# yenjane-dot/cognitive-aim-depth-estimation

Measured on NVIDIA B200. Metric: images/sec at 518x518 bf16, higher is better.
Workload: dtype bf16

## Files before the change

### cognitive_aim_depth_estimation_b200/csrc/common.cuh

```cuda
#pragma once

#include <cuda.h>
#include <cuda_bf16.h>
#include <cuda_runtime.h>
#include <stdint.h>
#include <stdio.h>

namespace ca {

enum : int {
  CA_OK = 0,
  CA_ERR_INVALID = 1,
  CA_ERR_CUDA = 2,
  CA_ERR_UNSUPPORTED = 3
};

__device__ __forceinline__ uint32_t smem_u32(const void* p) {
  return static_cast<uint32_t>(__cvta_generic_to_shared(p));
}
__device__ __forceinline__ uint32_t lane_id() { return threadIdx.x & 31u; }
__device__ __forceinline__ uint32_t warp_id() { return threadIdx.x >> 5; }

__device__ __forceinline__ bool elect_one_sync() {
  uint32_t pred;
// ... 163 lines not shown
    if ((++spins & 0x3fu) == 0 && (clock64() - t0) > 4000000000LL) {
      printf("[cogaim] mbarrier wait timed out: block (%d,%d,%d) thread %d bar@%u parity %u\n", blockIdx.x,
             blockIdx.y, blockIdx.z, threadIdx.x, smem_u32(bar), parity);
      __trap();
    }
  }
}

__device__ __forceinline__ void tma_prefetch_desc(const CUtensorMap* tm) {
  asm volatile("prefetch.tensormap [%0];" ::"l"(reinterpret_cast<uint64_t>(tm)) : "memory");
}
__device__ __forceinline__ void tma_load_2d(void* smem_dst, const CUtensorMap* tm, uint64_t* bar, int c0, int c1) {
  asm volatile(
      "cp.async.bulk.tensor.2d.shared::cluster.global.mbarrier::complete_tx::bytes [%0], [%1, {%3, %4}], [%2];"
      ::"r"(smem_u32(smem_dst)),
      "l"(reinterpret_cast<uint64_t>(tm)), "r"(smem_u32(bar)), "r"(c0), "r"(c1)
      : "memory");
}
__device__ __forceinline__ void tma_load_3d(void* smem_dst, const CUtensorMap* tm, uint64_t* bar, int c0, int c1,
                                            int c2) {
  asm volatile(
      "cp.async.bulk.tensor.3d.shared::cluster.global.mbarrier::complete_tx::bytes [%0], [%1, {%3, %4, %5}], [%2];"
      ::"r"(smem_u32(smem_dst)),
      "l"(reinterpret_cast<uint64_t>(tm)), "r"(smem_u32(bar)), "r"(c0), "r"(c1), "r"(c2)
      : "memory");
}

__device__ __forceinline__ void tma_reduce_add_2d(const CUtensorMap* tm, const void* smem_src, int c0, int c1) {
  asm volatile("cp.reduce.async.bulk.tensor.2d.global.shared::cta.add.tile.bulk_group [%0, {%2, %3}], [%1];" ::"l"(
                   reinterpret_cast<uint64_t>(tm)),
               "r"(smem_u32(smem_src)), "r"(c0), "r"(c1)
               : "memory");
}
__device__ __forceinline__ void bulk_commit_group() { asm volatile("cp.async.bulk.commit_group;" ::: "memory"); }
template <int kPending>
__device__ __forceinline__ void bulk_wait_group_read() {
  asm volatile("cp.async.bulk.wait_group.read %0;" ::"n"(kPending) : "memory");
}
template <int kPending>
__device__ __forceinline__ void bulk_wait_group() {
  asm volatile("cp.async.bulk.wait_group %0;" ::"n"(kPending) : "memory");
}

__device__ __forceinline__ void tmem_alloc(uint32_t* smem_result, uint32_t ncols) {
  asm volatile("tcgen05.alloc.cta_group::1.sync.aligned.shared::cta.b32 [%0], %1;" ::"r"(smem_u32(smem_result)),
               "r"(ncols)
               : "memory");
  asm volatile("tcgen05.relinquish_alloc_permit.cta_group::1.sync.aligned;" ::: "memory");
}
__device__ __forceinline__ void tmem_dealloc(uint32_t taddr, uint32_t ncols) {
  asm volatile("tcgen05.dealloc.cta_group::1.sync.aligned.b32 %0, %1;" ::"r"(taddr), "r"(ncols) : "memory");
}
__device__ __forceinline__ void tc_fence_before() { asm volatile("tcgen05.fence::before_thread_sync;" ::: "memory"); }
__device__ __forceinline__ void tc_fence_after() { asm volatile("tcgen05.fence::after_thread_sync;" ::: "memory"); }

__device__ __forceinline__ void umma_bf16(uint32_t tmem_d, uint64_t adesc, uint64_t bdesc, uint32_t idesc,
                                          uint32_t accumulate) {
  asm volatile(
      "{\n\t.reg .pred p;\n\t"
      "setp.ne.b32 p, %4, 0;\n\t"
      "tcgen05.mma.cta_group::1.kind::f16 [%0], %1, %2, %3, p;\n\t}"
      ::"r"(tmem_d),
      "l"(adesc), "l"(bdesc), "r"(idesc), "r"(accumulate)
      : "memory");
}
__device__ __forceinline__ void umma_bf16_ts(uint32_t tmem_d, uint32_t tmem_a, uint64_t bdesc, uint32_t idesc,
// ... 147 lines not shown
```

### cognitive_aim_depth_estimation_b200/csrc/gemm.cu

```cuda
#include "common.cuh"
#include "gemm.cuh"

#include <cuda_fp16.h>
#include "host.h"

#include <stdlib.h>

#ifndef CA_GEMM_RELEASE_ARRIVE
#define CA_GEMM_RELEASE_ARRIVE 0
#endif

namespace ca {

namespace {

constexpr int BM = 128;
constexpr int BK = 64;
constexpr int kNumEpiWarps = 8;
constexpr int kGemmThreads = (2 + kNumEpiWarps) * 32;
constexpr int kEpiStageBytes = 32 * 128;
__device__ __forceinline__ uint32_t epi_off(int r, int piece) { return r * 128 + ((piece ^ (r & 7)) << 4); }

template <int BN>
struct GemmCfg {
  static constexpr int kStages = (BN == 256) ? 4 : 6;
  static constexpr int kABytes = BM * BK * 2;
  static constexpr int kBBytes = BN * BK * 2;
  static constexpr int kStageBytes = kABytes + kBBytes;
  static constexpr int kTmemCols = 2 * BN;
  static constexpr int kStagingBytes = kNumEpiWarps * kEpiStageBytes;
  static constexpr int kSmemBytes = kStages * kStageBytes + kStagingBytes + 1024  + 256 ;
};

struct GemmKernelArgs {
  int M, N, K;
  int m_tiles, n_tiles, total_tiles;
  int w_batched;
  void* out;
  int ldo;
  long long out_batch_stride;
  const float* bias;
  const float* ls;
  const float* pos;
  int patches_per_img;
  float scale_log2;
  float* part_a;
  float* part_b;
  const float* col_max;
  const float* col_rinv;
  int partials;
  float2* ln_stats;
  int ln_slots;
  float ln_eps;
  __nv_bfloat16* shadow;
  int ld_shadow;
  int dbg;
};

__device__ __forceinline__ void gelu_erf2(float& x0, float& x1) {
  float s0, s1, p0, p1;
  fmul2(s0, s1, x0, x1, x0, x1);
  ffma2(p0, p1, s0, s1, 6.013480685629347e-11f, -5.644098521884189e-09f);
  ffma2v(p0, p1, p0, p1, s0, s1, 2.3467518417419342e-07f, 2.3467518417419342e-07f);
  ffma2v(p0, p1, p0, p1, s0, s1, -5.765378773503471e-06f, -5.765378773503471e-06f);
  ffma2v(p0, p1, p0, p1, s0, s1, 9.46131840464659e-05f, 9.46131840464659e-05f);
  ffma2v(p0, p1, p0, p1, s0, s1, -0.0011143309529870749f, -0.0011143309529870749f);
  ffma2v(p0, p1, p0, p1, s0, s1, 0.009830592200160027f, 0.009830592200160027f);
  ffma2v(p0, p1, p0, p1, s0, s1, -0.06636093556880951f, -0.06636093556880951f);
  ffma2v(p0, p1, p0, p1, s0, s1, 0.39890772104263306f, 0.39890772104263306f);
  const float phi0 = ffma_sat(p0, x0, 0.5f), phi1 = ffma_sat(p1, x1, 0.5f);
  fmul2(x0, x1, x0, x1, phi0, phi1);
}

__device__ __forceinline__ float ln_row_rstd(const GemmKernelArgs& p, int row) {
  if (row >= p.M) return 1.f;
  const float2* st = p.ln_stats + static_cast<size_t>(row) * p.ln_slots;
  const float inv_dim = 1.f / (128.f * p.ln_slots);
  float tot = 0.f, m2 = 0.f;
  for (int i = 0; i < p.ln_slots; ++i) {
    const float2 t = __ldg(st + i);
    tot += t.x;
    m2 += t.y;
  }
  const float mean = tot * inv_dim;
  for (int i = 0; i < p.ln_slots; ++i) {
    const float d = __ldg(st + i).x * (1.f / 128.f) - mean;
    m2 = fmaf(128.f * d, d, m2);
  }
  return rsqrtf(m2 * inv_dim + p.ln_eps);
}

template <int BN, int EPI>
__device__ __forceinline__ void epilogue_tile(const GemmKernelArgs& p, const CUtensorMap* tmap_x, uint32_t tmem_acc, int b,
                                              int mt, int nt, int quad, int half, uint8_t* stage, float rstd = 1.f) {
  constexpr int kSpan = BN / 2;
  const int lane = lane_id();
  const int row = mt * BM + quad * 32 + lane;
  const int col_base = nt * BN + half * kSpan;
  const bool row_ok = row < p.M;
  const uint32_t taddr = tmem_acc + (static_cast<uint32_t>(quad * 32) << 16) + static_cast<uint32_t>(half * kSpan);

  if constexpr (EPI == EPI_ROWSTATS) {
    constexpr int kSub = kSpan / 64;
    const uint32_t stage_s = smem_u32(stage);
#pragma unroll 1
    for (int sub = 0; sub < kSub; ++sub) {
      const int col_sub = col_base + sub * 64;
      const uint32_t taddr_sub = taddr + static_cast<uint32_t>(sub * 64);
      const bool full = col_sub + 64 <= p.N;
      float mx = -INFINITY;
#pragma unroll
      for (int c = 0; c < 64; c += 32) {
        uint32_t v[32];
        tmem_ld32(taddr_sub + c, v);
        tmem_ld_wait();
        if (full) {
          float m0 = __uint_as_float(v[0]), m1 = __uint_as_float(v[1]);
#pragma unroll
          for (int j = 2; j < 32; j += 2) {
            m0 = fmaxf(m0, __uint_as_float(v[j]));
            m1 = fmaxf(m1, __uint_as_float(v[j + 1]));
          }
          mx = fmaxf(mx, fmaxf(m0, m1));
        } else {
#pragma unroll
          for (int j = 0; j < 32; ++j)
            if (col_sub + c + j < p.N) mx = fmaxf(mx, __uint_as_float(v[j]));
// ... 59 lines not shown
      }
    }
    return;
  } else if constexpr (EPI == EPI_COLSUM) {
    const float* cmax = p.col_max + static_cast<size_t>(b) * p.N;
    const float* cinv = p.col_rinv + static_cast<size_t>(b) * p.N;
    float sum = 0.f;
#pragma unroll
    for (int c = 0; c < kSpan; c += 32) {
      uint32_t v[32];
      tmem_ld32(taddr + c, v);
      tmem_ld_wait();
#pragma unroll
      for (int j = 0; j < 32; ++j) {
        const int col = col_base + c + j;
        if (col < p.N) {
          const float s = __uint_as_float(v[j]) * p.scale_log2;
          sum += fast_exp2(s - __ldg(cmax + col)) * __ldg(cinv + col);
        }
      }
    }
    if (row_ok) {
      const size_t o = (static_cast<size_t>(b) * p.partials + nt * 2 + half) * p.M + row;
      p.part_a[o] = sum;
    }
    return;
  } else {
    const int lrow = lane >> 3;
    const int seg = lane & 7;
    const uint32_t stage_s = smem_u32(stage);
    if constexpr (EPI == EPI_BIAS_BF16 || EPI == EPI_GELU_BF16 || EPI == EPI_LN_BIAS_BF16 || EPI == EPI_LN_GELU_BF16) {
      constexpr bool kLn = (EPI == EPI_LN_BIAS_BF16 || EPI == EPI_LN_GELU_BF16);
      constexpr bool kGelu = (EPI == EPI_GELU_BF16 || EPI == EPI_LN_GELU_BF16);
#pragma unroll 1
      for (int c = 0; c < kSpan; c += 64) {
        const int col = col_base + c;
#pragma unroll
        for (int hh = 0; hh < 2; ++hh) {
          uint32_t v[32];
          tmem_ld32(taddr + c + 32 * hh, v);
          tmem_ld_wait();
          if (col < p.N) {
            const float4* b4 = reinterpret_cast<const float4*>(p.bias + col + 32 * hh);
#pragma unroll
            for (int j = 0; j < 4; ++j) {
              float a[8];
#pragma unroll
              for (int h = 0; h < 2; ++h) {
                const float4 t = __ldg(b4 + 2 * j + h);
                if constexpr (kLn) {
                  a[4 * h + 0] = fmaf(rstd, __uint_as_float(v[8 * j + 4 * h + 0]), t.x);
                  a[4 * h + 1] = fmaf(rstd, __uint_as_float(v[8 * j + 4 * h + 1]), t.y);
                  a[4 * h + 2] = fmaf(rstd, __uint_as_float(v[8 * j + 4 * h + 2]), t.z);
                  a[4 * h + 3] = fmaf(rstd, __uint_as_float(v[8 * j + 4 * h + 3]), t.w);
                } else {
                  a[4 * h + 0] = __uint_as_float(v[8 * j + 4 * h + 0]) + t.x;
                  a[4 * h + 1] = __uint_as_float(v[8 * j + 4 * h + 1]) + t.y;
                  a[4 * h + 2] = __uint_as_float(v[8 * j + 4 * h + 2]) + t.z;
                  a[4 * h + 3] = __uint_as_float(v[8 * j + 4 * h + 3]) + t.w;
                }
              }
              if constexpr (kGelu) {
#pragma unroll
                for (int i = 0; i < 8; i += 2) gelu_erf2(a[i], a[i + 1]);
              }
              uint4 w;
              w.x = pack_bf16x2(a[0], a[1]);
              w.y = pack_bf16x2(a[2], a[3]);
              w.z = pack_bf16x2(a[4], a[5]);
              w.w = pack_bf16x2(a[6], a[7]);
              sts128(stage_s + epi_off(lane, 4 * hh + j), w);
            }
          }
        }
        if (col < p.N) {
          __syncwarp();
          __nv_bfloat16* obase = reinterpret_cast<__nv_bfloat16*>(p.out) + static_cast<size_t>(b) * p.out_batch_stride +
                                 col + seg * 8;
#pragma unroll
          for (int i = 0; i < 8; ++i) {
            const int rr = lrow + 4 * i;
            const int grow = mt * BM + quad * 32 + rr;
            const uint4 w = lds128(stage_s + epi_off(rr, seg));
            if (grow < p.M) *reinterpret_cast<uint4*>(obase + static_cast<size_t>(grow) * p.ldo) = w;
          }
          __syncwarp();
        }
      }
    } else if constexpr (EPI == EPI_RESID_F32) {
      constexpr int kChunks = kSpan / 32;
#pragma unroll 1
      for (int g = 0; g < kChunks; ++g) {
        const int c = g * 32;
        uint32_t v[32];
        tmem_ld32(taddr + c, v);
        tmem_ld_wait();
        const int col = col_base + c;
        if (lane == 0) bulk_wait_group_read<0>();
        __syncwarp();
#pragma unroll
        for (int j = 0; j < 8; ++j) {
          const float4 t = __ldg(reinterpret_cast<const float4*>(p.bias + col) + j);
          const float4 l4 = __ldg(reinterpret_cast<const float4*>(p.ls + col) + j);
          sts128f(stage_s + epi_off(lane, j),
              make_float4(l4.x * (__uint_as_float(v[4 * j + 0]) + t.x), l4.y * (__uint_as_float(v[4 * j + 1]) + t.y),
                          l4.z * (__uint_as_float(v[4 * j + 2]) + t.z), l4.w * (__uint_as_float(v[4 * j + 3]) + t.w)));
        }
        fence_proxy_async_smem();
        __syncwarp();
        if (lane == 0) {
          tma_reduce_add_2d(tmap_x, stage, col, mt * BM + quad * 32);
          bulk_commit_group();
        }
      }
    } else {
#pragma unroll 1
      for (int c = 0; c < kSpan; c += 32) {
        uint32_t v[32];
        tmem_ld32(taddr + c, v);
        tmem_ld_wait();
        const int col = col_base + c;
        if (col < p.N) {
#pragma unroll
          for (int j = 0; j < 8; ++j) {
            float4 a = make_float4(__uint_as_float(v[4 * j + 0]), __uint_as_float(v[4 * j + 1]),
                                   __uint_as_float(v[4 * j + 2]), __uint_as_float(v[4 * j + 3]));
            if constexpr (EPI != EPI_F32) {
              const float4 t = __ldg(reinterpret_cast<const float4*>(p.bias + col) + j);
              a.x += t.x;
// ... 101 lines not shown
      uint32_t phase = 0;
      int acc = 0;
      uint32_t acc_phase = 0;
      for (int tile = blockIdx.x; tile < p.total_tiles; tile += gridDim.x) {
        mbar_wait(&acc_empty[acc], acc_phase ^ 1u);
        tc_fence_after();
        const uint32_t tmem_d = tmem_base + static_cast<uint32_t>(acc * BN);
        for (int kb = 0; kb < kblocks; ++kb) {
          mbar_wait(&full_bar[stage], phase);
          tc_fence_after();
          const uint64_t adesc = umma_smem_desc_sw128(smem_u32(smem_a + stage * Cfg::kABytes));
          const uint64_t bdesc = umma_smem_desc_sw128(smem_u32(smem_b + stage * Cfg::kBBytes));
#pragma unroll
          for (int k = 0; k < BK / 16; ++k) {
            umma_bf16(tmem_d, adesc + 2 * k, bdesc + 2 * k, idesc, (kb | k) != 0 ? 1u : 0u);
          }
          umma_commit(&empty_bar[stage]);
          if (++stage == Cfg::kStages) {
            stage = 0;
            phase ^= 1u;
          }
        }
        umma_commit(&acc_full[acc]);
        acc ^= 1;
        if (acc == 0) acc_phase ^= 1u;
      }
    }
  } else {
    const int e = warp - 2;
    const int quad = warp & 3;
    const int half = e >> 2;
    int acc = 0;
    uint32_t acc_phase = 0;
    for (int tile = blockIdx.x; tile < p.total_tiles; tile += gridDim.x) {
      const int nt = tile % p.n_tiles;
      const int rest = tile / p.n_tiles;
      const int mt = rest % p.m_tiles;
      const int b = rest / p.m_tiles;
      float rstd = 1.f;
      if constexpr (EPI == EPI_LN_BIAS_BF16 || EPI == EPI_LN_GELU_BF16) rstd = ln_row_rstd(p, mt * BM + quad * 32 + lane);
      mbar_wait(&acc_full[acc], acc_phase);
      tc_fence_after();
      epilogue_tile<BN, EPI>(p, &tmap_x, tmem_base + static_cast<uint32_t>(acc * BN), b, mt, nt, quad, half,
                             smem_stage + e * kEpiStageBytes, rstd);
      tc_fence_before();
      __syncwarp();
      if (lane == 0) mbar_arrive(&acc_empty[acc]);
      acc ^= 1;
      if (acc == 0) acc_phase ^= 1u;
    }
    if constexpr (EPI == EPI_RESID_F32) {
      if (lane == 0) bulk_wait_group<0>();
    }
  }

  tc_fence_before();
  __syncthreads();
  if (warp == 1) {
    tc_fence_after();
    tmem_dealloc(tmem_base, Cfg::kTmemCols);
  }
}

struct Gemm2Cfg {
  static constexpr int BN = 256;
  static constexpr int kStages = 6;
  static constexpr int kABytes = BM * BK * 2;
  static constexpr int kBBytes = (BN / 2) * BK * 2;
  static constexpr int kStageBytes = kABytes + kBBytes;
  static constexpr int kTmemCols = 2 * BN;
  static constexpr int kStagingBytes = kNumEpiWarps * kEpiStageBytes;
  static constexpr int kSmemBytes = kStages * kStageBytes + kStagingBytes + 1024 + 256;
};

template <int EPI>
__global__ void __cluster_dims__(2, 1, 1) __launch_bounds__(kGemmThreads, 1)
gemm2_tcgen05_kernel(const __grid_constant__ CUtensorMap tmap_a, const __grid_constant__ CUtensorMap tmap_w,
                     const __grid_constant__ CUtensorMap tmap_x, const GemmKernelArgs p) {
  using Cfg = Gemm2Cfg;
  constexpr int BN = Cfg::BN;
  constexpr bool kResidLn = (EPI == EPI_RESID_LN_F32);
  constexpr int n_stages = Cfg::kStages;
  constexpr int staging_bytes = Cfg::kStagingBytes;
  extern __shared__ uint8_t smem_raw[];
  uint8_t* smem = reinterpret_cast<uint8_t*>((reinterpret_cast<uintptr_t>(smem_raw) + 1023) & ~uintptr_t(1023));
  uint8_t* smem_a = smem;
  uint8_t* smem_b = smem + n_stages * Cfg::kABytes;
  uint8_t* smem_stage = smem + n_stages * Cfg::kStageBytes;
  uint64_t* bars = reinterpret_cast<uint64_t*>(smem_stage + staging_bytes);
  uint64_t* full_bar = bars;
  uint64_t* empty_bar = bars + Cfg::kStages;
  uint64_t* acc_full = bars + 2 * Cfg::kStages;
  uint64_t* acc_empty = acc_full + 2;
  uint32_t* tmem_slot = reinterpret_cast<uint32_t*>(acc_empty + 2);

  const int warp = warp_id();
  const int lane = lane_id();
  const uint32_t rank = cluster_ctarank();
  const int cluster_id = blockIdx.x >> 1;
  const int n_clusters = gridDim.x >> 1;
  const int kblocks = (p.K + BK - 1) / BK;

  if (warp == 0 && lane == 0) {
    tma_prefetch_desc(&tmap_a);
    tma_prefetch_desc(&tmap_w);
// ... 18 lines not shown
    if (lane == 0) {
      int stage = 0;
      uint32_t phase = 0;
      for (int tile = cluster_id; tile < p.total_tiles; tile += n_clusters) {
        const int nt = tile % p.n_tiles;
        const int rest = tile / p.n_tiles;
        const int mt2 = rest % p.m_tiles;
        const int b = rest / p.m_tiles;
        for (int kb = 0; kb < kblocks; ++kb) {
          mbar_wait(&empty_bar[stage], phase ^ 1u);
          const uint32_t leader_full = mapa_cluster(smem_u32(&full_bar[stage]), 0);
          const bool la = !(p.dbg & 2) || kb == 0, lb = !(p.dbg & 1) || kb == 0;
          const int mt_l = (p.dbg & 16) ? 0 : mt2, nt_l = (p.dbg & 16) ? 0 : nt;
          if (rank == 0)
            mbar_arrive_expect_tx(&full_bar[stage], 2 * ((la ? Cfg::kABytes : 0) + (lb ? Cfg::kBBytes : 0)));
          if (la) tma_load_3d_2sm(smem_a + stage * Cfg::kABytes, &tmap_a, leader_full, kb * BK, mt_l * 2 * BM + rank * BM, b);
          if (lb)
            tma_load_3d_2sm(smem_b + stage * Cfg::kBBytes, &tmap_w, leader_full, kb * BK, nt_l * BN + rank * (BN / 2),
                            p.w_batched ? b : 0);
          if (++stage == n_stages) {
            stage = 0;
            phase ^= 1u;
          }
        }
      }
    }
  } else if (warp == 1) {
    if (rank == 0 && lane == 0) {
      constexpr uint32_t idesc = umma_idesc_bf16(2 * BM, BN, 0, 0);
      int stage = 0;
      uint32_t phase = 0;
      int acc = 0;
      uint32_t acc_phase = 0;
      for (int tile = cluster_id; tile < p.total_tiles; tile += n_clusters) {
        mbar_wait(&acc_empty[acc], acc_phase ^ 1u);
        tc_fence_after();
        const uint32_t tmem_d = tmem_base + static_cast<uint32_t>(acc * BN);
        for (int kb = 0; kb < kblocks; ++kb) {
          mbar_wait(&full_bar[stage], phase);
          tc_fence_after();
          const uint64_t adesc = umma_smem_desc_sw128(smem_u32(smem_a + stage * Cfg::kABytes));
          const uint64_t bdesc = umma_smem_desc_sw128(smem_u32(smem_b + stage * Cfg::kBBytes));
#pragma unroll
          for (int k = 0; k < BK / 16; ++k) {
            umma_bf16_2sm(tmem_d, adesc + 2 * k, bdesc + 2 * k, idesc, (kb | k) != 0 ? 1u : 0u);
          }
          umma_commit_2sm(&empty_bar[stage], 3);
          if (++stage == n_stages) {
            stage = 0;
            phase ^= 1u;
          }
        }
        umma_commit_2sm(&acc_full[acc], 3);
        acc ^= 1;
        if (acc == 0) acc_phase ^= 1u;
      }
    }
  } else {
    const int e = warp - 2;
    const int quad = warp & 3;
    const int half = e >> 2;
    int acc = 0;
    uint32_t acc_phase = 0;
    if constexpr (kResidLn) {
      const int lrow = lane >> 3, seg = lane & 7;
      const uint32_t stage_s = smem_u32(smem_stage + e * kEpiStageBytes);
      const int my_tiles = cluster_id < p.total_tiles ? (p.total_tiles - cluster_id + n_clusters - 1) / n_clusters : 0;
      const int total_chunks = my_tiles * 4;
      auto tile_origin = [&](int i, int& col0, int& row0, int& nt) {
        const int tile = cluster_id + i * n_clusters;
        nt = tile % p.n_tiles;
        const int mt2 = (tile / p.n_tiles) % p.m_tiles;
        col0 = nt * BN + half * 128;
        row0 = (mt2 * 2 + static_cast<int>(rank)) * BM + quad * 32;
      };
      float* const xbase = reinterpret_cast<float*>(p.out);
      float4 old[8];
      int n_col0 = 0, n_row0 = 0, n_nt = 0;
      auto load_piece = [&](int s, int i) {
        const int row = n_row0 + lrow + 4 * i;
        old[i] = row < p.M ? *reinterpret_cast<const float4*>(xbase + static_cast<size_t>(row) * p.ldo + n_col0 + (s & 3) * 32 + seg * 4)
                           : make_float4(0.f, 0.f, 0.f, 0.f);
      };
      if (total_chunks > 0) {
        tile_origin(0, n_col0, n_row0, n_nt);
#pragma unroll
// ... 50 lines not shown
          float4 n;
          fadd2v(n.x, n.y, old[i].x, old[i].y, d.x, d.y);
          fadd2v(n.z, n.w, old[i].z, old[i].w, d.z, d.w);
          if (more) load_piece(s + 1, i);
          if (row < p.M) {
            *reinterpret_cast<float4*>(xbase + static_cast<size_t>(row) * p.ldo + col + seg * 4) = n;
            *reinterpret_cast<uint2*>(p.shadow + static_cast<size_t>(row) * p.ld_shadow + col + seg * 4) =
                make_uint2(pack_bf16x2(n.x, n.y), pack_bf16x2(n.z, n.w));
          }
          rs[i] += (n.x + n.y) + (n.z + n.w);
          rq[i] = fmaf(n.x, n.x, fmaf(n.y, n.y, fmaf(n.z, n.z, fmaf(n.w, n.w, rq[i]))));
        }
        __syncwarp();
        if (g == 3) {
#pragma unroll
          for (int i = 0; i < 8; ++i) {
#pragma unroll
            for (int o = 1; o < 8; o <<= 1) {
              rs[i] += __shfl_xor_sync(0xffffffffu, rs[i], o);
              rq[i] += __shfl_xor_sync(0xffffffffu, rq[i], o);
            }
          }
          if (seg == 0) {
#pragma unroll
            for (int i = 0; i < 8; ++i) {
              const int row = row0 + lrow + 4 * i;
              if (row < p.M)
                p.ln_stats[static_cast<size_t>(row) * p.ln_slots + nt * 2 + half] =
                    make_float2(rs[i], fmaxf(rq[i] - rs[i] * rs[i] * (1.f / 128.f), 0.f));
            }
          }
        }
      }
    } else
    for (int tile = cluster_id; tile < p.total_tiles; tile += n_clusters) {
      const int nt = tile % p.n_tiles;
      const int rest = tile / p.n_tiles;
      const int mt = (rest % p.m_tiles) * 2 + static_cast<int>(rank);
      const int b = rest / p.m_tiles;
      float rstd = 1.f;
      if constexpr (EPI == EPI_LN_BIAS_BF16 || EPI == EPI_LN_GELU_BF16) rstd = ln_row_rstd(p, mt * BM + quad * 32 + lane);
      mbar_wait(&acc_full[acc], acc_phase);
      tc_fence_after();
      epilogue_tile<BN, EPI>(p, &tmap_x, tmem_base + static_cast<uint32_t>(acc * BN), b, mt, nt, quad, half,
                             smem_stage + e * kEpiStageBytes, rstd);
      tc_fence_before();
      __syncwarp();
#if CA_GEMM_RELEASE_ARRIVE
      if (lane == 0) mbar_arrive_cluster(mapa_cluster(smem_u32(&acc_empty[acc]), 0));
#else
      if (lane == 0) mbar_arrive_remote(mapa_cluster(smem_u32(&acc_empty[acc]), 0));
#endif
      acc ^= 1;
      if (acc == 0) acc_phase ^= 1u;
    }
    if constexpr (EPI == EPI_RESID_F32) {
      if (lane == 0) bulk_wait_group<0>();
    }
  }

  tc_fence_before();
  cluster_sync_all();
  if (warp == 1) {
    tc_fence_after();
    tmem_dealloc_2sm(tmem_base, Cfg::kTmemCols);
  }
}

template <int EPI>
int launch_inst2(const CUtensorMap& ta, const CUtensorMap& tw, const CUtensorMap& tx, const GemmKernelArgs& ka,
                 cudaStream_t stream) {
  auto kern = gemm2_tcgen05_kernel<EPI>;
  const int smem = Gemm2Cfg::kSmemBytes;
  static PerDeviceOnce configured;
  CA_TRY(configured.run([&]() -> int {
    CA_CUDA(cudaFuncSetAttribute(kern, cudaFuncAttributeMaxDynamicSharedMemorySize, Gemm2Cfg::kSmemBytes));
    return 0;
  }));
  const int max_clusters = sm_count() / 2;
  const int clusters = ka.total_tiles < max_clusters ? ka.total_tiles : max_clusters;
  CA_TRY(launch_kernel(kern, dim3(2 * clusters), dim3(kGemmThreads), smem, stream, ta, tw, tx, ka));
  CA_CUDA(cudaGetLastError());
  return 0;
}

template <int BN, int EPI>
int launch_inst(const CUtensorMap& ta, const CUtensorMap& tw, const CUtensorMap& tx, const GemmKernelArgs& ka,
                cudaStream_t stream) {
  using Cfg = GemmCfg<BN>;
  auto kern = gemm_tcgen05_kernel<BN, EPI>;
  static PerDeviceOnce configured;
  CA_TRY(configured.run([&]() -> int {
    CA_CUDA(cudaFuncSetAttribute(kern, cudaFuncAttributeMaxDynamicSharedMemorySize, Cfg::kSmemBytes));
    return 0;
  }));
  int grid = ka.total_tiles < sm_count() ? ka.total_tiles : sm_count();
  CA_TRY(launch_kernel(kern, dim3(grid), dim3(kGemmThreads), Cfg::kSmemBytes, stream, ta, tw, tx, ka));
  CA_CUDA(cudaGetLastError());
  return 0;
}

}

int gemm_launch(const GemmArgs& a, cudaStream_t stream) {
  CA_REQUIRE(a.A && a.W, "gemm: null operand");
  CA_REQUIRE(a.M > 0 && a.N > 0 && a.K > 0 && a.batch > 0, "gemm: non-positive dimension");
  CA_REQUIRE(a.lda % 8 == 0 && a.ldw % 8 == 0, "gemm: lda/ldw must be multiples of 8 elements (16 B) for TMA");
  CA_REQUIRE(a.K <= a.lda && a.K <= a.ldw, "gemm: K exceeds a leading dimension");
  const bool stats = (a.epilogue == EPI_ROWSTATS || a.epilogue == EPI_COLSUM);
  static const bool force_1cta = getenv("CA_GEMM_1CTA") != nullptr;
  const bool resid_ln = a.epilogue == EPI_RESID_LN_F32;
  const bool ln_in = a.epilogue == EPI_LN_BIAS_BF16 || a.epilogue == EPI_LN_GELU_BF16;
  const bool pair = (!force_1cta || resid_ln) && a.epilogue != EPI_COLSUM;
  const int bn = (stats && !pair) ? 128 : 256;
  if (!stats) {
    CA_REQUIRE(a.N % 32 == 0, "gemm: N must be a multiple of 32 for the dense epilogues");
    const bool bf16_out = a.epilogue == EPI_BIAS_BF16 || a.epilogue == EPI_GELU_BF16 || ln_in;
    CA_REQUIRE(!bf16_out || a.N % 64 == 0, "gemm: the bf16 epilogues need N % 64 == 0");
    CA_REQUIRE(a.out != nullptr, "gemm: null output");
    CA_REQUIRE(a.epilogue == EPI_F32 || a.bias != nullptr, "gemm: null bias");
    const int vec = bf16_out ? 8 : 4;
    CA_REQUIRE(a.ldo % vec == 0, "gemm: ldo must keep rows 16-byte aligned");
    const bool resid = a.epilogue == EPI_RESID_F32 || resid_ln;
    CA_REQUIRE(!resid || a.ls != nullptr, "gemm: null LayerScale");
    CA_REQUIRE(!resid || a.N % 256 == 0, "gemm: the residual epilogues need N % 256 == 0");
    CA_REQUIRE(!(ln_in || resid_ln) || (a.ln_stats != nullptr && a.ln_slots > 0 && a.batch == 1),
               "gemm: the LayerNorm-folding epilogues need a statistics buffer and are not batched");
    CA_REQUIRE(!ln_in || (a.K == 128 * a.ln_slots && a.ln_eps > 0.f), "gemm: EPI_LN_* need K == 128 * ln_slots and eps > 0");
    CA_REQUIRE(!resid_ln || (a.shadow != nullptr && a.N == 128 * a.ln_slots && a.ld_shadow % 8 == 0 &&
                             (reinterpret_cast<uintptr_t>(a.shadow) & 15) == 0),
               "gemm: EPI_RESID_LN_F32 needs a 16-byte aligned bf16 shadow and N == 128 * ln_slots");
    CA_REQUIRE(a.epilogue != EPI_PATCH_F32 || (a.pos != nullptr && a.patches_per_img > 0), "gemm: null pos-embed");
  } else {
    CA_REQUIRE(a.part_a != nullptr, "gemm: null partial buffer");
    CA_REQUIRE(a.epilogue != EPI_ROWSTATS || a.part_b != nullptr, "gemm: null partial-sum buffer");
    CA_REQUIRE(a.epilogue != EPI_COLSUM || (a.col_max && a.col_rinv), "gemm: null column statistics");
    CA_REQUIRE(a.epilogue != EPI_ROWSTATS || a.out == nullptr || (a.ldo % 64 == 0 && a.ldo >= a.N),
               "gemm: the exponential matrix needs a leading dimension that is a multiple of 64 and >= N");
  }

  CUtensorMap ta, tw;
  const long long abs = a.batch > 1 ? a.a_batch_stride : static_cast<long long>(a.M) * a.lda;
  CA_REQUIRE(abs % 8 == 0, "gemm: A batch stride must be a multiple of 8 elements");
  CA_TRY(make_tmap_3d(&ta, a.A, a.batch, a.M, a.K, a.lda, abs, BM));
  const bool wb = a.batch > 1 && a.w_batch_stride != 0;
  const long long wbs = wb ? a.w_batch_stride : static_cast<long long>(a.N) * a.ldw;
  CA_REQUIRE(wbs % 8 == 0, "gemm: W batch stride must be a multiple of 8 elements");
  CA_TRY(make_tmap_3d(&tw, a.W, wb ? a.batch : 1, a.N, a.K, a.ldw, wbs, pair ? bn / 2 : bn));

  CUtensorMap tx = ta;
  if (a.epilogue == EPI_RESID_F32 || resid_ln) {
    CA_REQUIRE(a.batch == 1, "gemm: the residual epilogue is not batched");
    CA_REQUIRE(a.ldo % 4 == 0 && (reinterpret_cast<uintptr_t>(a.out) & 15) == 0, "gemm: residual rows must be 16-byte aligned");
    CA_TRY(make_tmap_f32_2d(&tx, a.out, a.M, a.N, a.ldo, 32));
  }

  GemmKernelArgs ka;
  ka.M = a.M;
  ka.N = a.N;
  ka.K = a.K;
  ka.m_tiles = pair ? (a.M + 2 * BM - 1) / (2 * BM) : (a.M + BM - 1) / BM;
  ka.n_tiles = (a.N + bn - 1) / bn;
  if (stats && bn == 128) ka.n_tiles = (ka.n_tiles + 1) & ~1;
  ka.total_tiles = ka.m_tiles * ka.n_tiles * a.batch;
  ka.w_batched = wb ? 1 : 0;
  ka.out = a.out;
  ka.ldo = a.ldo;
  ka.out_batch_stride = a.out_batch_stride;
  ka.bias = a.bias;
  ka.ls = a.ls;
  ka.pos = a.pos;
  ka.patches_per_img = a.patches_per_img;
  ka.scale_log2 = a.scale_log2;
  ka.part_a = a.part_a;
  ka.part_b = a.part_b;
  ka.col_max = a.col_max;
  ka.col_rinv = a.col_rinv;
  ka.partials = gemm_stats_partials(a.N);
  ka.ln_stats = reinterpret_cast<float2*>(a.ln_stats);
  ka.ln_slots = a.ln_slots;
  ka.ln_eps = a.ln_eps;
  ka.shadow = a.shadow;
  ka.ld_shadow = a.ld_shadow;
  static const int dbg = getenv("CA_GEMM_DEBUG") ? atoi(getenv("CA_GEMM_DEBUG")) : 0;
  ka.dbg = dbg;

  if (pair) {
    switch (a.epilogue) {
      case EPI_BIAS_BF16: return launch_inst2<EPI_BIAS_BF16>(ta, tw, tx, ka, stream);
      case EPI_GELU_BF16: return launch_inst2<EPI_GELU_BF16>(ta, tw, tx, ka, stream);
      case EPI_RESID_F32: return launch_inst2<EPI_RESID_F32>(ta, tw, tx, ka, stream);
      case EPI_PATCH_F32: return launch_inst2<EPI_PATCH_F32>(ta, tw, tx, ka, stream);
      case EPI_F32: return launch_inst2<EPI_F32>(ta, tw, tx, ka, stream);
      case EPI_ROWSTATS: return launch_inst2<EPI_ROWSTATS>(ta, tw, tx, ka, stream);
      case EPI_LN_BIAS_BF16: return launch_inst2<EPI_LN_BIAS_BF16>(ta, tw, tx, ka, stream);
      case EPI_LN_GELU_BF16: return launch_inst2<EPI_LN_GELU_BF16>(ta, tw, tx, ka, stream);
      case EPI_RESID_LN_F32: return launch_inst2<EPI_RESID_LN_F32>(ta, tw, tx, ka, stream);
      default: return invalid("gemm: unknown epilogue");
    }
  }
  switch (a.epilogue) {
    case EPI_BIAS_BF16: return launch_inst<256, EPI_BIAS_BF16>(ta, tw, tx, ka, stream);
    case EPI_GELU_BF16: return launch_inst<256, EPI_GELU_BF16>(ta, tw, tx, ka, stream);
    case EPI_RESID_F32: return launch_inst<256, EPI_RESID_F32>(ta, tw, tx, ka, stream);
    case EPI_PATCH_F32: return launch_inst<256, EPI_PATCH_F32>(ta, tw, tx, ka, stream);
    case EPI_F32: return launch_inst<256, EPI_F32>(ta, tw, tx, ka, stream);
    case EPI_LN_BIAS_BF16: return launch_inst<256, EPI_LN_BIAS_BF16>(ta, tw, tx, ka, stream);
    case EPI_LN_GELU_BF16: return launch_inst<256, EPI_LN_GELU_BF16>(ta, tw, tx, ka, stream);
    case EPI_ROWSTATS: return launch_inst<128, EPI_ROWSTATS>(ta, tw, tx, ka, stream);
    case EPI_COLSUM: return launch_inst<128, EPI_COLSUM>(ta, tw, tx, ka, stream);
    default: return invalid("gemm: unknown epilogue");
  }
}

}
```

Before: 2651.

## Store GELU bf16 GEMM epilogue via TMA with smem-staged prefetched bias

For the GELU bf16 epilogues, the output now goes out through a 3D TMA tensor store from swizzled shared-memory staging instead of per-thread global stores. The bias for each tile is prefetched one tile ahead into shared memory, replacing repeated global bias loads in the inner loop. The aim is to cut LSU and global-store pressure in the epilogue and overlap output writes with the next tile's work. In exchange it adds a named barrier per tile, extra shared memory, and bulk-group waits before staging is reused. Compile-time tracing instrumentation and optional direct-store variants, off by default, are also added.

```diff
diff --git a/cognitive_aim_depth_estimation_b200/csrc/common.cuh b/cognitive_aim_depth_estimation_b200/csrc/common.cuh
--- a/cognitive_aim_depth_estimation_b200/csrc/common.cuh
+++ b/cognitive_aim_depth_estimation_b200/csrc/common.cuh
@@ -219,6 +219,12 @@
                "r"(smem_u32(smem_src)), "r"(c0), "r"(c1)
                : "memory");
 }
+__device__ __forceinline__ void tma_store_3d(const CUtensorMap* tm, const void* smem_src, int c0, int c1, int c2) {
+  asm volatile("cp.async.bulk.tensor.3d.global.shared::cta.tile.bulk_group [%0, {%2, %3, %4}], [%1];" ::"l"(
+                   reinterpret_cast<uint64_t>(tm)),
+               "r"(smem_u32(smem_src)), "r"(c0), "r"(c1), "r"(c2)
+               : "memory");
+}
 __device__ __forceinline__ void bulk_commit_group() { asm volatile("cp.async.bulk.commit_group;" ::: "memory"); }
 template <int kPending>
 __device__ __forceinline__ void bulk_wait_group_read() {
diff --git a/cognitive_aim_depth_estimation_b200/csrc/gemm.cu b/cognitive_aim_depth_estimation_b200/csrc/gemm.cu
--- a/cognitive_aim_depth_estimation_b200/csrc/gemm.cu
+++ b/cognitive_aim_depth_estimation_b200/csrc/gemm.cu
@@ -4,10 +4,14 @@
 #include <cuda_fp16.h>
 #include "host.h"
 
+#include <stdio.h>
 #include <stdlib.h>
 
 #ifndef CA_GEMM_RELEASE_ARRIVE
 #define CA_GEMM_RELEASE_ARRIVE 0
+#endif
+#ifndef CA_GEMM_TRACE
+#define CA_GEMM_TRACE 0
 #endif
 
 namespace ca {
@@ -29,7 +33,8 @@
   static constexpr int kStageBytes = kABytes + kBBytes;
   static constexpr int kTmemCols = 2 * BN;
   static constexpr int kStagingBytes = kNumEpiWarps * kEpiStageBytes;
-  static constexpr int kSmemBytes = kStages * kStageBytes + kStagingBytes + 1024  + 256 ;
+  static constexpr int kBiasBytes = BN * 4;
+  static constexpr int kSmemBytes = kStages * kStageBytes + kStagingBytes + 1024  + 256  + kBiasBytes;
 };
 
 struct GemmKernelArgs {
@@ -55,7 +60,24 @@
   __nv_bfloat16* shadow;
   int ld_shadow;
   int dbg;
+  long long* trace;
 };
+
+constexpr int kTraceTiles = 64;
+constexpr int kTraceSlots = 32;
+#if CA_GEMM_TRACE
+#define GEMM_TRACE(i, slot, value)                                                                       \
+  do {                                                                                                   \
+    if (p.trace && cluster_id == 0 && rank == 0 && lane == 0 && (i) < kTraceTiles) p.trace[(i) * kTraceSlots + (slot)] = (value); \
+  } while (0)
+#define GEMM_TRACE_LD()      \
+  do {                       \
+    if (t_ld) *t_ld = clock64(); \
+  } while (0)
+#else
+#define GEMM_TRACE(i, slot, value) do {} while (0)
+#define GEMM_TRACE_LD() do {} while (0)
+#endif
 
 __device__ __forceinline__ void gelu_erf2(float& x0, float& x1) {
   float s0, s1, p0, p1;
@@ -90,9 +112,36 @@
   return rsqrtf(m2 * inv_dim + p.ln_eps);
 }
 
+#ifndef CA_GEMM_TMA_ALL
+#define CA_GEMM_TMA_ALL 0
+#endif
+#ifndef CA_GEMM_BF16_DIRECT
+#define CA_GEMM_BF16_DIRECT 0
+#endif
+__host__ __device__ constexpr bool gelu_bf16_epi(int epi) {
+  return epi == EPI_GELU_BF16 || epi == EPI_LN_GELU_BF16 ||
+         (CA_GEMM_TMA_ALL && (epi == EPI_BIAS_BF16 || epi == EPI_LN_BIAS_BF16));
+}
+template <int EPI>
+constexpr bool kBiasStaged = gelu_bf16_epi(EPI);
+
+template <int BN>
+__device__ __forceinline__ float bias_of_tile(const GemmKernelArgs& p, int tile, int e, int lane) {
+  static_assert(BN == 32 * kNumEpiWarps, "one bias value per epilogue thread");
+  if (tile >= p.total_tiles) return 0.f;
+  const int col = (tile % p.n_tiles) * BN + e * 32 + lane;
+  return col < p.N ? __ldg(p.bias + col) : 0.f;
+}
+__device__ __forceinline__ void bias_stage_store(uint32_t s_bias, int e, int lane, float v) {
+  named_bar_sync(1, kNumEpiWarps * 32);
+  asm volatile("st.shared.f32 [%0], %1;" ::"r"(s_bias + 4u * (e * 32 + lane)), "f"(v) : "memory");
+  named_bar_sync(1, kNumEpiWarps * 32);
+}
+
 template <int BN, int EPI>
 __device__ __forceinline__ void epilogue_tile(const GemmKernelArgs& p, const CUtensorMap* tmap_x, uint32_t tmem_acc, int b,
-                                              int mt, int nt, int quad, int half, uint8_t* stage, float rstd = 1.f) {
+                                              int mt, int nt, int quad, int half, uint8_t* stage, float rstd = 1.f,
+                                              uint32_t s_bias = 0, long long* t_ld = nullptr) {
   constexpr int kSpan = BN / 2;
   const int lane = lane_id();
   const int row = mt * BM + quad * 32 + lane;
@@ -218,16 +267,71 @@
     if constexpr (EPI == EPI_BIAS_BF16 || EPI == EPI_GELU_BF16 || EPI == EPI_LN_BIAS_BF16 || EPI == EPI_LN_GELU_BF16) {
       constexpr bool kLn = (EPI == EPI_LN_BIAS_BF16 || EPI == EPI_LN_GELU_BF16);
       constexpr bool kGelu = (EPI == EPI_GELU_BF16 || EPI == EPI_LN_GELU_BF16);
+      if constexpr (gelu_bf16_epi(EPI)) {
 #pragma unroll 1
-      for (int c = 0; c < kSpan; c += 64) {
-        const int col = col_base + c;
-#pragma unroll
-        for (int hh = 0; hh < 2; ++hh) {
+        for (int c = 0; c < kSpan; c += 64) {
+          const int col = col_base + c;
+          uint32_t v[2][32];
+          tmem_ld32(taddr + c, v[0]);
+          tmem_ld32(taddr + c + 32, v[1]);
+          tmem_ld_wait();
+          GEMM_TRACE_LD();
+          if (col < p.N) {
+            if (lane == 0) bulk_wait_group_read<0>();
+            __syncwarp();
+#pragma unroll
+            for (int hh = 0; hh < 2; ++hh) {
+#pragma unroll
+              for (int j = 0; j < 4; ++j) {
+                float a[8];
+#pragma unroll
+                for (int h = 0; h < 2; ++h) {
+                  const float4 t = lds128f(s_bias + 4 * (half * kSpan + c + 32 * hh + 8 * j + 4 * h));
+                  const uint32_t* vv = v[hh];
+                  if constexpr (kLn) {
+                    a[4 * h + 0] = fmaf(rstd, __uint_as_float(vv[8 * j + 4 * h + 0]), t.x);
+                    a[4 * h + 1] = fmaf(rstd, __uint_as_float(vv[8 * j + 4 * h + 1]), t.y);
+                    a[4 * h + 2] = fmaf(rstd, __uint_as_float(vv[8 * j + 4 * h + 2]), t.z);
+                    a[4 * h + 3] = fmaf(rstd, __uint_as_float(vv[8 * j + 4 * h + 3]), t.w);
+                  } else {
+                    a[4 * h + 0] = __uint_as_float(vv[8 * j + 4 * h + 0]) + t.x;
+                    a[4 * h + 1] = __uint_as_float(vv[8 * j + 4 * h + 1]) + t.y;
+                    a[4 * h + 2] = __uint_as_float(vv[8 * j + 4 * h + 2]) + t.z;
+                    a[4 * h + 3] = __uint_as_float(vv[8 * j + 4 * h + 3]) + t.w;
+                  }
+                }
+                if constexpr (kGelu) {
+#pragma unroll
+                  for (int i = 0; i < 8; i += 2) gelu_erf2(a[i], a[i + 1]);
+                }
+                uint4 w;
+                w.x = pack_bf16x2(a[0], a[1]);
+                w.y = pack_bf16x2(a[2], a[3]);
+                w.z = pack_bf16x2(a[4], a[5]);
+                w.w = pack_bf16x2(a[6], a[7]);
+                sts128(stage_s + epi_off(lane, 4 * hh + j), w);
+              }
+            }
+            fence_proxy_async_smem();
+            __syncwarp();
+            if (lane == 0) {
+              tma_store_3d(tmap_x, stage, col, mt * BM + quad * 32, b);
+              bulk_commit_group();
+            }
+          }
+        }
+      } else if constexpr (CA_GEMM_BF16_DIRECT) {
+#pragma unroll 1
+        for (int c = 0; c < kSpan; c += 32) {
+          const int col = col_base + c;
           uint32_t v[32];
-          tmem_ld32(taddr + c + 32 * hh, v);
+          tmem_ld32(taddr + c, v);
           tmem_ld_wait();
+          GEMM_TRACE_LD();
           if (col < p.N) {
-            const float4* b4 = reinterpret_cast<const float4*>(p.bias + col + 32 * hh);
+            const float4* b4 = reinterpret_cast<const float4*>(p.bias + col);
+            __nv_bfloat16* orow = reinterpret_cast<__nv_bfloat16*>(p.out) + static_cast<size_t>(b) * p.out_batch_stride +
+                                  static_cast<size_t>(row) * p.ldo + col;
 #pragma unroll
             for (int j = 0; j < 4; ++j) {
               float a[8];
@@ -246,31 +350,67 @@
                   a[4 * h + 3] = __uint_as_float(v[8 * j + 4 * h + 3]) + t.w;
                 }
               }
-              if constexpr (kGelu) {
-#pragma unroll
-                for (int i = 0; i < 8; i += 2) gelu_erf2(a[i], a[i + 1]);
-              }
               uint4 w;
               w.x = pack_bf16x2(a[0], a[1]);
               w.y = pack_bf16x2(a[2], a[3]);
               w.z = pack_bf16x2(a[4], a[5]);
               w.w = pack_bf16x2(a[6], a[7]);
-              sts128(stage_s + epi_off(lane, 4 * hh + j), w);
+              if (row_ok) *reinterpret_cast<uint4*>(orow + 8 * j) = w;
             }
           }
         }
-        if (col < p.N) {
-          __syncwarp();
-          __nv_bfloat16* obase = reinterpret_cast<__nv_bfloat16*>(p.out) + static_cast<size_t>(b) * p.out_batch_stride +
-                                 col + seg * 8;
-#pragma unroll
-          for (int i = 0; i < 8; ++i) {
-            const int rr = lrow + 4 * i;
-            const int grow = mt * BM + quad * 32 + rr;
-            const uint4 w = lds128(stage_s + epi_off(rr, seg));
-            if (grow < p.M) *reinterpret_cast<uint4*>(obase + static_cast<size_t>(grow) * p.ldo) = w;
-          }
-          __syncwarp();
+      } else {
+#pragma unroll 1
+        for (int c = 0; c < kSpan; c += 64) {
+          const int col = col_base + c;
+#pragma unroll
+          for (int hh = 0; hh < 2; ++hh) {
+            uint32_t v[32];
+            tmem_ld32(taddr + c + 32 * hh, v);
+            tmem_ld_wait();
+            GEMM_TRACE_LD();
+            if (col < p.N) {
+              const float4* b4 = reinterpret_cast<const float4*>(p.bias + col + 32 * hh);
+#pragma unroll
+              for (int j = 0; j < 4; ++j) {
+                float a[8];
+#pragma unroll
+                for (int h = 0; h < 2; ++h) {
+                  const float4 t = __ldg(b4 + 2 * j + h);
+                  if constexpr (kLn) {
+                    a[4 * h + 0] = fmaf(rstd, __uint_as_float(v[8 * j + 4 * h + 0]), t.x);
+                    a[4 * h + 1] = fmaf(rstd, __uint_as_float(v[8 * j + 4 * h + 1]), t.y);
+                    a[4 * h + 2] = fmaf(rstd, __uint_as_float(v[8 * j + 4 * h + 2]), t.z);
+                    a[4 * h + 3] = fmaf(rstd, __uint_as_float(v[8 * j + 4 * h + 3]), t.w);
+                  } else {
+                    a[4 * h + 0] = __uint_as_float(v[8 * j + 4 * h + 0]) + t.x;
+                    a[4 * h + 1] = __uint_as_float(v[8 * j + 4 * h + 1]) + t.y;
+                    a[4 * h + 2] = __uint_as_float(v[8 * j + 4 * h + 2]) + t.z;
+                    a[4 * h + 3] = __uint_as_float(v[8 * j + 4 * h + 3]) + t.w;
+                  }
+                }
+                uint4 w;
+                w.x = pack_bf16x2(a[0], a[1]);
+                w.y = pack_bf16x2(a[2], a[3]);
+                w.z = pack_bf16x2(a[4], a[5]);
+                w.w = pack_bf16x2(a[6], a[7]);
+                sts128(stage_s + epi_off(lane, 4 * hh + j), w);
+              }
+            }
+          }
+          if (col < p.N) {
+            __syncwarp();
+            __nv_bfloat16* obase = reinterpret_cast<__nv_bfloat16*>(p.out) + static_cast<size_t>(b) * p.out_batch_stride +
+                                   col + seg * 8;
+#pragma unroll
+            for (int i = 0; i < 8; ++i) {
+              const int rr = lrow + 4 * i;
+              const int grow = mt * BM + quad * 32 + rr;
+              const uint4 w = lds128(stage_s + epi_off(rr, seg));
+              if (grow < p.M) *reinterpret_cast<uint4*>(obase + static_cast<size_t>(grow) * p.ldo) = w;
+            }
+            __syncwarp();
+          }
         }
       }
     } else if constexpr (EPI == EPI_RESID_F32) {
@@ -281,6 +421,7 @@
         uint32_t v[32];
         tmem_ld32(taddr + c, v);
         tmem_ld_wait();
+        GEMM_TRACE_LD();
         const int col = col_base + c;
         if (lane == 0) bulk_wait_group_read<0>();
         __syncwarp();
@@ -448,24 +589,31 @@
     const int half = e >> 2;
     int acc = 0;
     uint32_t acc_phase = 0;
+    const uint32_t s_bias = smem_u32(smem_stage + Cfg::kStagingBytes + 256);
+    float bias_next = 0.f;
+    if constexpr (kBiasStaged<EPI>) bias_next = bias_of_tile<BN>(p, blockIdx.x, e, lane);
     for (int tile = blockIdx.x; tile < p.total_tiles; tile += gridDim.x) {
       const int nt = tile % p.n_tiles;
       const int rest = tile / p.n_tiles;
       const int mt = rest % p.m_tiles;
       const int b = rest / p.m_tiles;
+      if constexpr (kBiasStaged<EPI>) {
+        bias_stage_store(s_bias, e, lane, bias_next);
+        bias_next = bias_of_tile<BN>(p, tile + gridDim.x, e, lane);
+      }
       float rstd = 1.f;
       if constexpr (EPI == EPI_LN_BIAS_BF16 || EPI == EPI_LN_GELU_BF16) rstd = ln_row_rstd(p, mt * BM + quad * 32 + lane);
       mbar_wait(&acc_full[acc], acc_phase);
       tc_fence_after();
       epilogue_tile<BN, EPI>(p, &tmap_x, tmem_base + static_cast<uint32_t>(acc * BN), b, mt, nt, quad, half,
-                             smem_stage + e * kEpiStageBytes, rstd);
+                             smem_stage + e * kEpiStageBytes, rstd, s_bias);
       tc_fence_before();
       __syncwarp();
       if (lane == 0) mbar_arrive(&acc_empty[acc]);
       acc ^= 1;
       if (acc == 0) acc_phase ^= 1u;
     }
-    if constexpr (EPI == EPI_RESID_F32) {
+    if constexpr (EPI == EPI_RESID_F32 || (gelu_bf16_epi(EPI))) {
       if (lane == 0) bulk_wait_group<0>();
     }
   }
@@ -486,7 +634,8 @@
   static constexpr int kStageBytes = kABytes + kBBytes;
   static constexpr int kTmemCols = 2 * BN;
   static constexpr int kStagingBytes = kNumEpiWarps * kEpiStageBytes;
-  static constexpr int kSmemBytes = kStages * kStageBytes + kStagingBytes + 1024 + 256;
+  static constexpr int kBiasBytes = BN * 4;
+  static constexpr int kSmemBytes = kStages * kStageBytes + kStagingBytes + 1024 + 256 + kBiasBytes;
 };
 
 template <int EPI>
@@ -571,12 +720,23 @@
       uint32_t phase = 0;
       int acc = 0;
       uint32_t acc_phase = 0;
-      for (int tile = cluster_id; tile < p.total_tiles; tile += n_clusters) {
+      int it = 0;
+      for (int tile = cluster_id; tile < p.total_tiles; tile += n_clusters, ++it) {
+        GEMM_TRACE(it, 0, clock64());
         mbar_wait(&acc_empty[acc], acc_phase ^ 1u);
+        GEMM_TRACE(it, 1, clock64());
         tc_fence_after();
         const uint32_t tmem_d = tmem_base + static_cast<uint32_t>(acc * BN);
+        long long full_wait = 0;
+        (void)full_wait;
         for (int kb = 0; kb < kblocks; ++kb) {
+#if CA_GEMM_TRACE
+          const long long w0 = clock64();
           mbar_wait(&full_bar[stage], phase);
+          full_wait += clock64() - w0;
+#else
+          mbar_wait(&full_bar[stage], phase);
+#endif
           tc_fence_after();
           const uint64_t adesc = umma_smem_desc_sw128(smem_u32(smem_a + stage * Cfg::kABytes));
           const uint64_t bdesc = umma_smem_desc_sw128(smem_u32(smem_b + stage * Cfg::kBBytes));
@@ -584,6 +744,8 @@
           for (int k = 0; k < BK / 16; ++k) {
             umma_bf16_2sm(tmem_d, adesc + 2 * k, bdesc + 2 * k, idesc, (kb | k) != 0 ? 1u : 0u);
           }
+          if (kb == 0) GEMM_TRACE(it, 2, clock64());
+          if (kb == kblocks - 1) GEMM_TRACE(it, 3, clock64());
           umma_commit_2sm(&empty_bar[stage], 3);
           if (++stage == n_stages) {
             stage = 0;
@@ -591,6 +753,7 @@
           }
         }
         umma_commit_2sm(&acc_full[acc], 3);
+        GEMM_TRACE(it, 4, full_wait);
         acc ^= 1;
         if (acc == 0) acc_phase ^= 1u;
       }
@@ -707,29 +870,42 @@
           }
         }
       }
-    } else
-    for (int tile = cluster_id; tile < p.total_tiles; tile += n_clusters) {
-      const int nt = tile % p.n_tiles;
-      const int rest = tile / p.n_tiles;
-      const int mt = (rest % p.m_tiles) * 2 + static_cast<int>(rank);
-      const int b = rest / p.m_tiles;
-      float rstd = 1.f;
-      if constexpr (EPI == EPI_LN_BIAS_BF16 || EPI == EPI_LN_GELU_BF16) rstd = ln_row_rstd(p, mt * BM + quad * 32 + lane);
-      mbar_wait(&acc_full[acc], acc_phase);
-      tc_fence_after();
-      epilogue_tile<BN, EPI>(p, &tmap_x, tmem_base + static_cast<uint32_t>(acc * BN), b, mt, nt, quad, half,
-                             smem_stage + e * kEpiStageBytes, rstd);
-      tc_fence_before();
-      __syncwarp();
+    } else {
+      const uint32_t s_bias = smem_u32(smem_stage + staging_bytes + 256);
+      float bias_next = 0.f;
+      if constexpr (kBiasStaged<EPI>) bias_next = bias_of_tile<BN>(p, cluster_id, e, lane);
+      int it = 0;
+      for (int tile = cluster_id; tile < p.total_tiles; tile += n_clusters, ++it) {
+        const int nt = tile % p.n_tiles;
+        const int rest = tile / p.n_tiles;
+        const int mt = (rest % p.m_tiles) * 2 + static_cast<int>(rank);
+        const int b = rest / p.m_tiles;
+        if constexpr (kBiasStaged<EPI>) {
+          bias_stage_store(s_bias, e, lane, bias_next);
+          bias_next = bias_of_tile<BN>(p, tile + n_clusters, e, lane);
+        }
+        float rstd = 1.f;
+        if constexpr (EPI == EPI_LN_BIAS_BF16 || EPI == EPI_LN_GELU_BF16) rstd = ln_row_rstd(p, mt * BM + quad * 32 + lane);
+        mbar_wait(&acc_full[acc], acc_phase);
+        tc_fence_after();
+        GEMM_TRACE(it, 8 + 3 * e, clock64());
+        long long t_ld = 0;
+        epilogue_tile<BN, EPI>(p, &tmap_x, tmem_base + static_cast<uint32_t>(acc * BN), b, mt, nt, quad, half,
+                               smem_stage + e * kEpiStageBytes, rstd, s_bias, CA_GEMM_TRACE ? &t_ld : nullptr);
+        GEMM_TRACE(it, 8 + 3 * e + 1, t_ld);
+        GEMM_TRACE(it, 8 + 3 * e + 2, clock64());
+        tc_fence_before();
+        __syncwarp();
 #if CA_GEMM_RELEASE_ARRIVE
-      if (lane == 0) mbar_arrive_cluster(mapa_cluster(smem_u32(&acc_empty[acc]), 0));
+        if (lane == 0) mbar_arrive_cluster(mapa_cluster(smem_u32(&acc_empty[acc]), 0));
 #else
-      if (lane == 0) mbar_arrive_remote(mapa_cluster(smem_u32(&acc_empty[acc]), 0));
+        if (lane == 0) mbar_arrive_remote(mapa_cluster(smem_u32(&acc_empty[acc]), 0));
 #endif
-      acc ^= 1;
-      if (acc == 0) acc_phase ^= 1u;
-    }
-    if constexpr (EPI == EPI_RESID_F32) {
+        acc ^= 1;
+        if (acc == 0) acc_phase ^= 1u;
+      }
+    }
+    if constexpr (EPI == EPI_RESID_F32 || (gelu_bf16_epi(EPI))) {
       if (lane == 0) bulk_wait_group<0>();
     }
   }
@@ -774,6 +950,52 @@
   CA_CUDA(cudaGetLastError());
   return 0;
 }
+
+#if CA_GEMM_TRACE
+int print_trace(const long long* d_trace, const GemmKernelArgs& ka, int epi, cudaStream_t stream) {
+  static long long tr[kTraceTiles * kTraceSlots];
+  CA_CUDA(cudaStreamSynchronize(stream));
+  CA_CUDA(cudaMemcpy(tr, d_trace, sizeof(tr), cudaMemcpyDeviceToHost));
+  const int max_clusters = sm_count() / 2;
+  const int clusters = ka.total_tiles < max_clusters ? ka.total_tiles : max_clusters;
+  int n = (ka.total_tiles + clusters - 1) / clusters;
+  n = n < kTraceTiles ? n : kTraceTiles;
+  const long long t0 = tr[0];
+  fprintf(stderr, "[gemm trace] M %d N %d K %d epi %d: %d tiles on %d clusters, cluster 0 has %d; clk since its first acc_empty wait\n",
+          ka.M, ka.N, ka.K, epi, ka.total_tiles, clusters, n);
+  fprintf(stderr, "  tile | mma: empty_wait -> got  first_kb  last_kb  full_wait | epi: acc_full min..max  last_ld max  last_store max\n");
+  double s_empty = 0, s_issue = 0, s_full = 0, s_period = 0, s_epi = 0, s_ld = 0, s_lat = 0;
+  int cnt = 0;
+  for (int i = 0; i < n; ++i) {
+    const long long* t = tr + i * kTraceSlots;
+    long long af_min = t[8], af_max = t[8], ld_max = t[9], st_max = t[10];
+    for (int e = 1; e < kNumEpiWarps; ++e) {
+      const long long* w = t + 8 + 3 * e;
+      af_min = w[0] < af_min ? w[0] : af_min;
+      af_max = w[0] > af_max ? w[0] : af_max;
+      ld_max = w[1] > ld_max ? w[1] : ld_max;
+      st_max = w[2] > st_max ? w[2] : st_max;
+    }
+    fprintf(stderr, "  %4d | %9lld -> %9lld %9lld %9lld %9lld | %9lld..%9lld %9lld %9lld\n", i, t[0] - t0, t[1] - t0, t[2] - t0,
+            t[3] - t0, t[4], af_min - t0, af_max - t0, ld_max - t0, st_max - t0);
+    if (i >= 2 && i + 1 < n) {
+      s_empty += t[1] - t[0];
+      s_issue += t[3] - t[1];
+      s_full += t[4];
+      s_period += tr[(i + 1) * kTraceSlots + 1] - t[1];
+      s_epi += st_max - af_min;
+      s_ld += ld_max - af_min;
+      s_lat += af_min - t[3];
+      ++cnt;
+    }
+  }
+  if (cnt > 0)
+    fprintf(stderr, "  mean over %d tiles (clk): tile period %.0f | mma: acc_empty wait %.0f, issue span %.0f (full_bar waits %.0f) | "
+                    "last K block issued -> acc_full %.0f | epi: acc_full -> last ld %.0f, -> last store %.0f\n",
+            cnt, s_period / cnt, s_empty / cnt, s_issue / cnt, s_full / cnt, s_lat / cnt, s_ld / cnt, s_epi / cnt);
+  return 0;
+}
+#endif
 
 }
 
@@ -828,6 +1050,14 @@
     CA_REQUIRE(a.batch == 1, "gemm: the residual epilogue is not batched");
     CA_REQUIRE(a.ldo % 4 == 0 && (reinterpret_cast<uintptr_t>(a.out) & 15) == 0, "gemm: residual rows must be 16-byte aligned");
     CA_TRY(make_tmap_f32_2d(&tx, a.out, a.M, a.N, a.ldo, 32));
+  } else if (gelu_bf16_epi(a.epilogue)) {
+    CA_REQUIRE((reinterpret_cast<uintptr_t>(a.out) & 15) == 0, "gemm: bf16 output rows must be 16-byte aligned");
+    CA_REQUIRE(a.batch == 1 || a.out_batch_stride % 8 == 0, "gemm: the bf16 output batch stride must be a multiple of 8 elements");
+    const uint64_t obs = a.batch > 1 ? static_cast<uint64_t>(a.out_batch_stride) : static_cast<uint64_t>(a.M) * a.ldo;
+    const uint64_t dims[3] = {static_cast<uint64_t>(a.N), static_cast<uint64_t>(a.M), static_cast<uint64_t>(a.batch)};
+    const uint64_t strides[2] = {static_cast<uint64_t>(a.ldo) * 2, obs * 2};
+    const uint32_t box[3] = {64, 32, 1};
+    CA_TRY(make_tmap_bf16_sw128(&tx, a.out, 3, dims, strides, box));
   }
 
   GemmKernelArgs ka;
@@ -859,20 +1089,35 @@
   ka.ld_shadow = a.ld_shadow;
   static const int dbg = getenv("CA_GEMM_DEBUG") ? atoi(getenv("CA_GEMM_DEBUG")) : 0;
   ka.dbg = dbg;
+  ka.trace = nullptr;
 
   if (pair) {
+#if CA_GEMM_TRACE
+    static long long* d_trace = nullptr;
+    const bool tracing = getenv("CA_GEMM_TRACE") != nullptr;
+    if (tracing) {
+      if (!d_trace) CA_CUDA(cudaMalloc(&d_trace, sizeof(long long) * kTraceTiles * kTraceSlots));
+      CA_CUDA(cudaMemsetAsync(d_trace, 0, sizeof(long long) * kTraceTiles * kTraceSlots, stream));
+      ka.trace = d_trace;
+    }
+#endif
+    int rc;
     switch (a.epilogue) {
-      case EPI_BIAS_BF16: return launch_inst2<EPI_BIAS_BF16>(ta, tw, tx, ka, stream);
-      case EPI_GELU_BF16: return launch_inst2<EPI_GELU_BF16>(ta, tw, tx, ka, stream);
-      case EPI_RESID_F32: return launch_inst2<EPI_RESID_F32>(ta, tw, tx, ka, stream);
-      case EPI_PATCH_F32: return launch_inst2<EPI_PATCH_F32>(ta, tw, tx, ka, stream);
-      case EPI_F32: return launch_inst2<EPI_F32>(ta, tw, tx, ka, stream);
-      case EPI_ROWSTATS: return launch_inst2<EPI_ROWSTATS>(ta, tw, tx, ka, stream);
-      case EPI_LN_BIAS_BF16: return launch_inst2<EPI_LN_BIAS_BF16>(ta, tw, tx, ka, stream);
-      case EPI_LN_GELU_BF16: return launch_inst2<EPI_LN_GELU_BF16>(ta, tw, tx, ka, stream);
-      case EPI_RESID_LN_F32: return launch_inst2<EPI_RESID_LN_F32>(ta, tw, tx, ka, stream);
+      case EPI_BIAS_BF16: rc = launch_inst2<EPI_BIAS_BF16>(ta, tw, tx, ka, stream); break;
+      case EPI_GELU_BF16: rc = launch_inst2<EPI_GELU_BF16>(ta, tw, tx, ka, stream); break;
+      case EPI_RESID_F32: rc = launch_inst2<EPI_RESID_F32>(ta, tw, tx, ka, stream); break;
+      case EPI_PATCH_F32: rc = launch_inst2<EPI_PATCH_F32>(ta, tw, tx, ka, stream); break;
+      case EPI_F32: rc = launch_inst2<EPI_F32>(ta, tw, tx, ka, stream); break;
+      case EPI_ROWSTATS: rc = launch_inst2<EPI_ROWSTATS>(ta, tw, tx, ka, stream); break;
+      case EPI_LN_BIAS_BF16: rc = launch_inst2<EPI_LN_BIAS_BF16>(ta, tw, tx, ka, stream); break;
+      case EPI_LN_GELU_BF16: rc = launch_inst2<EPI_LN_GELU_BF16>(ta, tw, tx, ka, stream); break;
+      case EPI_RESID_LN_F32: rc = launch_inst2<EPI_RESID_LN_F32>(ta, tw, tx, ka, stream); break;
       default: return invalid("gemm: unknown epilogue");
     }
+#if CA_GEMM_TRACE
+    if (rc == 0 && tracing) CA_TRY(print_trace(d_trace, ka, a.epilogue, stream));
+#endif
+    return rc;
   }
   switch (a.epilogue) {
     case EPI_BIAS_BF16: return launch_inst<256, EPI_BIAS_BF16>(ta, tw, tx, ka, stream);
```

New measurement: 2668, median of 6. Within noise of the previous version (+0.6%).
